# MishaLaskin/vqvae

Hardware: AMD Instinct MI355X
Metric: images/sec VQ-VAE forward (32x32x3, K=512, D=64) (higher is better)
Workload: dtype f32 (fp32 in/out/accumulate; conv products from two fp16 terms per operand, <= 2^-21 rel per product); 1 GPU; BASELINE config 3: full HIP path (Encoder+VQ+Decoder), 32x32x3, K=512, D=64; per_gpu_batch=4096, global_batch=4096, K=512, D=64, parallelism=batch-sharded replicas x1, no collective

## Files before the change

### vqvae_amd/csrc/conv_fused.hip

```cpp
#include "conv_host.h"

namespace vqvae {
#ifndef VQVAE_MID_SHFL_BPERMUTE
constexpr bool kSwz = true;
#else
constexpr bool kSwz = false;
#endif
#ifndef CRP_NW
#define CRP_NW 4
#endif
#ifndef CRP_MINW
#define CRP_MINW 2
#endif
struct DecHeadArgs {
    FrontConv fc;
    const u32x4 *w1img, *w2img;
    const int *hdr1, *hdr2;
    int flags;
    float *out;
    int *out_amax;
};
template <int NT3, bool VQ = false, bool GATHER = false, bool ZEOUT = false, bool DECHEAD = false>
__global__ __launch_bounds__(CRP_NW * 64, CRP_MINW) void conv_res_pair8_h2_kernel(const float *__restrict__ in, FrontConv fc,
                                                                   const u32x4 *__restrict__ w1img, const u32x4 *__restrict__ w2img,
                                                                   float *__restrict__ out, int B, int flags,
                                                                   const int *__restrict__ hdr1, const int *__restrict__ hdr2,
                                                                   const int *__restrict__ in_amax, int *__restrict__ out_amax,
                                                                   const u32x4 *__restrict__ w3img, const int *__restrict__ hdr3,
                                                                   const float *__restrict__ bias3, float *__restrict__ out3,
                                                                   int *__restrict__ zero_buf, int zero_n, VqFuse vq, DecHeadArgs dh) {
    static_assert(!DECHEAD || (VQ && !GATHER && !ZEOUT), "the decoder's head continues the quantizing instance");
    static_assert(NT3 == 0 || NT3 == 1 || NT3 == 2 || NT3 == 4, "the 1x1 post conv streams through NT3 weight stages of 16 KiB");
    static_assert(!VQ || (NT3 == 2 && CRP_NW == 4), "the fused quantizer takes the 64-channel z_e of four images per workgroup");
    constexpr int NT2 = 4, C = 128, MT = 2, PX = 64, HP = PX + 1, PLANE = HP * 2;
    constexpr int TILE4 = 2 * 2 * PLANE;
    constexpr int RBUF = 4 * HP;
    __shared__ u32x4 As_all[CRP_NW * TILE4];
    constexpr int WBUF = 18 * 64;
    const int nvq = VQ ? (vq.K32 >> 7) : 0;
    int NSTAGE = 18 + NT3 + nvq;
    FrontConv fcc = fc;
    const u32x4 *w1c = w1img, *w2c = w2img;
    __shared__ u32x4 Wb_all[2 * WBUF];
    __shared__ __attribute__((aligned(16))) unsigned char vq_tab_all[VQ ? CRP_NW * 1040 : 16];
    __shared__ int vq_hist_s[VQ ? 1024 : 1];
    __shared__ __attribute__((aligned(16))) float dw_s[288 + 32 * (NT3 > 0 ? NT3 : 1)];
    for (int i = threadIdx.x; i < 288 + 32 * NT3; i += CRP_NW * 64)
        dw_s[i] = i < 128 ? h2_dw(fc.hdr)[i] : (i < 160 ? h2_dw(hdr1)[i - 128] : (i < 288 ? h2_dw(hdr2)[i - 160] : h2_dw(hdr3)[i - 288]));
    __shared__ double vq_red_s[VQ ? CRP_NW : 1];
    if constexpr (VQ) {
        for (int i = threadIdx.x; i < vq.K; i += CRP_NW * 64) vq_hist_s[i] = 0;
    }
    const int tid = threadIdx.x, wave = tid >> 6;
    int lane, l31, h;
    u32x4 *As;
    float *Hs;
    unsigned dma_lane;
    int spx[MT];
    unsigned tapok[MT], tapok0[MT];
    const bool relu_out = flags & kFlagReluOut;
    constexpr int cpt = C >> 5;

    const long long img = (long long)blockIdx.x * CRP_NW + wave;
    const bool img_ok = img < B;
    if (zero_buf && blockIdx.x == 0)
        for (int i = tid; i < zero_n; i += CRP_NW * 64) zero_buf[i] = 0;

    auto lane_setup = [&](int t_id) {
        lane = t_id & 63;
        l31 = lane & 31;
        h = lane >> 5;
        As = As_all + (t_id >> 6) * TILE4;
        Hs = reinterpret_cast<float *>(As);
        dma_lane = (unsigned)lane * 16u;
#pragma unroll
        for (int mt = 0; mt < MT; ++mt) {
            spx[mt] = 32 * mt + l31;
            const int y = spx[mt] >> 3, x = spx[mt] & 7;
            unsigned m = 0;
#pragma unroll
            for (int t = 0; t < 9; ++t) {
                const int yy = y + t / 3 - 1, xx = x + t % 3 - 1;
                if (yy >= 0 && yy < 8 && xx >= 0 && xx < 8) m |= 1u << t;
            }
            tapok[mt] = m;
        }
    };
    lane_setup(tid);
    auto front_masks = [&]() {
#pragma unroll
        for (int mt = 0; mt < MT; ++mt) {
            const int y = spx[mt] >> 3, x = spx[mt] & 7;
            unsigned m0 = 0;
#pragma unroll
            for (int t = 0; t < 9; ++t) {
                const int y0 = y + (int)((fcc.dym >> (4 * t)) & 15) - 8, x0 = x + (int)((fcc.dxm >> (4 * t)) & 15) - 8;
                if (y0 >= 0 && y0 < 8 && x0 >= 0 && x0 < 8) m0 |= 1u << t;
            }
            tapok0[mt] = m0;
        }
    };
    front_masks();

    f32x16 Y[MT][NT2];
    const int wave_u = __builtin_amdgcn_readfirstlane(wave);
    auto dma = [&](const u32x4 *src_uniform, u32x4 *dst_piece) {
        const unsigned lds = __builtin_amdgcn_readfirstlane((unsigned)(unsigned long long)(__attribute__((address_space(3))) char *)(char *)dst_piece);
        asm volatile("s_mov_b32 m0, %2\n\ts_nop 0\n\tglobal_load_lds_dwordx4 %0, %1" ::"v"(dma_lane), "s"(src_uniform), "s"(lds) : "memory");
    };
    auto dma_slice = [&](int sl, int buf) {
        const u32x4 *base = w1c + (size_t)(sl >> 1) * 256 + (sl & 1) * 64;
        for (int p = wave_u; p < 18; p += CRP_NW)
            dma(base + (size_t)(p >> 1) * cpt * 256 + (p & 1) * 128, Wb_all + buf * WBUF + p * 64);
    };
    auto dma_linear = [&](const u32x4 *src, int buf) {
#pragma unroll
        for (int j = 0; j < 16 / CRP_NW; ++j) dma(src + (wave_u * (16 / CRP_NW) + j) * 64, Wb_all + buf * WBUF + (wave_u * (16 / CRP_NW) + j) * 64);
    };
    auto dma_stage = [&](int k, int buf) {
        if (VQ && k >= 18 + NT3) {
            const int j = k - (18 + NT3);
            dma_linear(reinterpret_cast<const u32x4 *>(vq.imgf) + (size_t)j * 1024, buf);
            if (wave_u == 0) dma(reinterpret_cast<const u32x4 *>(vq.seeds) + (size_t)j * 32, Wb_all + buf * WBUF + 16 * 64);
        }
        else if (k >= 18) dma_linear(w3img + (size_t)(k - 18) * 1024, buf);
        else if (k % 9 == 8) dma_linear(w2c, buf);
        else dma_slice(k % 9, buf);
    };
    auto dma_wait_sync = [&]() {
        asm volatile("s_waitcnt vmcnt(0)" ::: "memory");
        __syncthreads();
    };
    float ymax = 0.0f;
    int wstage = 0;
    f32x4 zr[2][8];
    f32x16(&Yo)[MT][NT2] = Y;
    float &ymax_o = ymax;
    int &wstage_o = wstage;
    auto front = [&](auto FZ) __attribute__((always_inline)) {
        constexpr bool FROMZ = decltype(FZ)::value;
        const FrontConv &fc = fcc;
        f32x16 Y[MT][NT2];
        float ymax = 0.0f;
        int wstage = 0;
        const int cpt0 = FROMZ ? 2 : fc.Cin >> 5;
        const float *src = in + ((size_t)(img_ok ? img : 0) * PX + lane) * fc.Cin;
        bool gbad = false;
        if constexpr (GATHER) {
            const long long k = vq.idx[(size_t)(img_ok ? img : 0) * PX + lane];
            gbad = k < 0 || k >= vq.K;
            src = in + (size_t)(gbad ? 0 : k) * fc.Cin;
        }
        const bool gany = GATHER && __builtin_amdgcn_ballot_w64(gbad) != 0;
        f32x4 raw[8];
        auto load_raw0 = [&](int cc) {
            if constexpr (FROMZ) {
#pragma unroll
                for (int j = 0; j < 8; ++j) raw[j] = cc == 0 ? zr[0][j] : zr[1][j];
                return;
            }
#pragma unroll
            for (int j = 0; j < 8; ++j) raw[j] = *reinterpret_cast<const f32x4 *>(src + 32 * cc + 4 * j);
            if (gany) {
                const float qn = __builtin_nanf("");
#pragma unroll
                for (int j = 0; j < 8; ++j) if (gbad) raw[j] = f32x4{qn, qn, qn, qn};
            }
        };
        float m = 0.0f;
        const int given = (!FROMZ && in_amax && img_ok) ? in_amax[img] : -1;
        auto fold_raw = [&]() {
#pragma unroll
            for (int j = 0; j < 8; ++j)
                m = fmaxf(m, fmaxf(fmaxf(__builtin_fabsf(raw[j].x), __builtin_fabsf(raw[j].y)), fmaxf(__builtin_fabsf(raw[j].z), __builtin_fabsf(raw[j].w))));
        };
        if constexpr (FROMZ) {
            load_raw0(0); fold_raw();
            load_raw0(1); fold_raw();
        } else if (given >= 0) m = __int_as_float(given);
        else for (int cc = 0; cc < cpt0; ++cc) {
            load_raw0(cc);
            fold_raw();
        }
        const int kx = wave_scale_exp<kSwz>(img_ok ? m : 0.0f);
        const float xs = __builtin_ldexpf(1.0f, kx), d0 = __builtin_ldexpf(1.0f, -kx);
#pragma unroll
        for (int mt = 0; mt < MT; ++mt)
#pragma unroll
            for (int nt = 0; nt < NT2; ++nt)
#pragma unroll
                for (int r = 0; r < 16; ++r) Y[mt][nt][r] = 0.0f;
        if (lane < 8) As[(lane >> 1) * PLANE + (lane & 1) * HP + PX] = u32x4{0, 0, 0, 0};
        auto dma_front = [&](int cc, int tap, int buf) {
            const u32x4 *base = fc.wimg + (size_t)(tap * cpt0 + cc) * (NT2 * 256);
#pragma unroll
            for (int j = 0; j < 16 / CRP_NW; ++j) {
                const int p = wave_u * (16 / CRP_NW) + j;
                dma(base + (p >> 2) * 256 + ((p >> 1) & 1) * 64 + (p & 1) * 128, Wb_all + buf * WBUF + p * 64);
            }
        };
        load_raw0(0);
        dma_front(0, 0, 0);
        for (int cc = 0; cc < cpt0; ++cc) {
            __builtin_amdgcn_wave_barrier();
            u32x4 *dst = As + lane;
#pragma unroll
            for (int t = 0; t < 2; ++t)
#pragma unroll
                for (int hh = 0; hh < 2; ++hh) {
                    u32x4 t1, t2;
                    split8_h(raw[4 * hh + 2 * t], raw[4 * hh + 2 * t + 1], xs, t1, t2);
                    dst[(t * 2 + 0) * PLANE + hh * HP] = t1;
                    dst[(t * 2 + 1) * PLANE + hh * HP] = t2;
                }
            lds_order_wave();
#pragma unroll 1
            for (int tap = 0; tap < 9; ++tap, ++wstage) {
                const int shift = ((int)((fc.dym >> (4 * tap)) & 15) - 8) * 8 + ((int)((fc.dxm >> (4 * tap)) & 15) - 8);
                u32x4 X[2][MT][2];
#pragma unroll
                for (int t = 0; t < 2; ++t)
#pragma unroll
                    for (int mt = 0; mt < MT; ++mt) {
                        const int p = ((tapok0[mt] >> tap) & 1u) ? spx[mt] + shift : PX;
                        const u32x4 *ap = As + (t * 2) * PLANE + h * HP + p;
                        X[t][mt][0] = ap[0];
                        X[t][mt][1] = ap[PLANE];
                    }
                if (!FROMZ && tap == 1 && cc + 1 < cpt0) {
                    asm volatile("s_waitcnt vmcnt(8)" ::: "memory");
                    __syncthreads();
                } else dma_wait_sync();
                if (tap + 1 < 9) dma_front(cc, tap + 1, (wstage + 1) & 1);
                else if (cc + 1 < cpt0) dma_front(cc + 1, 0, (wstage + 1) & 1);
                else dma_stage(0, (wstage + 1) & 1);
                if (tap == 0 && cc + 1 < cpt0) load_raw0(FROMZ ? 1 : cc + 1);
                const u32x4 *wt = Wb_all + (wstage & 1) * WBUF + lane;
                u32x4 Wc0 = wt[0], Wc1 = wt[64];
#pragma unroll
                for (int g = 0; g < 8; ++g) {
                    const int t = g >> 2, nt = g & 3;
                    u32x4 Wn0 = Wc0, Wn1 = Wc1;
                    if (g + 1 < 8) {
                        const u32x4 *bp = wt + (((g + 1) & 3) * 4 + ((g + 1) >> 2) * 2) * 64;
                        Wn0 = bp[0];
                        Wn1 = bp[64];
                    }
                    __builtin_amdgcn_sched_barrier(0);
                    prod3x2t(X[t][0][0], X[t][0][1], X[t][1][0], X[t][1][1], Wc0, Wc1, Y[0][nt], Y[1][nt]);
                    __builtin_amdgcn_sched_barrier(0);
                    Wc0 = Wn0;
                    Wc1 = Wn1;
                }
            }
        }
#pragma unroll
        for (int nt = 0; nt < NT2; ++nt)
#pragma unroll
            for (int g = 0; g < 4; ++g) {
                f32x4 bv = {0.0f, 0.0f, 0.0f, 0.0f};
                if (fc.bias) bv = *reinterpret_cast<const f32x4 *>(fc.bias + nt * 32 + 8 * g + 4 * h);
                const f32x4 dv = h2_dw4(dw_s, nt * 32, g, h, d0);
#pragma unroll
                for (int mt = 0; mt < MT; ++mt)
#pragma unroll
                    for (int q = 0; q < 4; q += 2)
                        SCALE2_BIAS_RELU2(Y[mt][nt][4 * g + q], Y[mt][nt][4 * g + q + 1], dv[q], dv[q + 1], bv[q], bv[q + 1], ymax);
            }
        lds_order_wave();
#pragma unroll
        for (int mt = 0; mt < MT; ++mt)
#pragma unroll
            for (int nt = 0; nt < NT2; ++nt) Yo[mt][nt] = Y[mt][nt];
        ymax_o = ymax;
        wstage_o = wstage;
    };
    front(std::false_type{});

    auto stage_sync = [&](int k) -> const u32x4 * {
        dma_wait_sync();
        if (k + 1 < NSTAGE) dma_stage(k + 1, (wstage + k + 1) & 1);
        return Wb_all + ((wstage + k) & 1) * WBUF + lane;
    };
    f32x16 acc1[MT];
    auto taps = [&](const u32x4 *wb, const u32x4 *pl) {
        u32x4 Xc[MT][2], Wc[2];
        auto ld = [&](int tap, u32x4(&X)[MT][2], u32x4(&W)[2]) {
            const int shift = (tap / 3 - 1) * 8 + (tap % 3 - 1);
#pragma unroll
            for (int mt = 0; mt < MT; ++mt) {
                const int p = ((tapok[mt] >> tap) & 1u) ? spx[mt] + shift : PX;
                X[mt][0] = pl[p];
                X[mt][1] = pl[p + HP * 2];
            }
            W[0] = wb[tap * 128];
            W[1] = wb[tap * 128 + 64];
        };
        ld(0, Xc, Wc);
#pragma unroll
        for (int tap = 0; tap < 9; ++tap) {
            u32x4 Xn[MT][2], Wn[2];
            if (tap + 1 < 9) ld(tap + 1, Xn, Wn);
            __builtin_amdgcn_sched_barrier(0);
            prod3x2t(Xc[0][0], Xc[0][1], Xc[1][0], Xc[1][1], Wc[0], Wc[1], acc1[0], acc1[1]);
            __builtin_amdgcn_sched_barrier(0);
            if (tap + 1 < 9) {
#pragma unroll
                for (int mt = 0; mt < MT; ++mt) { Xc[mt][0] = Xn[mt][0]; Xc[mt][1] = Xn[mt][1]; }
                Wc[0] = Wn[0]; Wc[1] = Wn[1];
            }
        }
    };
    auto put_planes = [&](int buf, const u32x4(&T1)[MT][2], const u32x4(&T2)[MT][2], int t) {
        u32x4 *pb = As + buf * RBUF + h * HP + l31;
#pragma unroll
        for (int mt = 0; mt < MT; ++mt) {
            pb[32 * mt] = T1[mt][t];
            pb[32 * mt + 2 * HP] = T2[mt][t];
        }
    };
    auto layer = [&](auto LT, bool relu_after) __attribute__((always_inline)) {
        constexpr int LI = decltype(LT)::value;
        const int kx = wave_scale_exp<kSwz>(img_ok ? ymax : 0.0f);
        const float xscale = __builtin_ldexpf(1.0f, kx), d1 = __builtin_ldexpf(1.0f, -kx);
#pragma unroll
        for (int mt = 0; mt < MT; ++mt)
#pragma unroll
            for (int r = 0; r < 16; ++r) acc1[mt][r] = 0.0f;
        u32x4 T1[MT][2], T2[MT][2];
#pragma unroll
        for (int mt = 0; mt < MT; ++mt) acc_to_ksteps(Y[mt][0], xscale, T1[mt], T2[mt]);
        __builtin_amdgcn_wave_barrier();
        put_planes(0, T1, T2, 0);
#pragma unroll
        for (int c = 0; c < NT2; ++c) {
            __builtin_amdgcn_wave_barrier();
            put_planes(1, T1, T2, 1);
            lds_order_wave();
            taps(stage_sync(9 * LI + 2 * c), As + h * HP);
            if (c + 1 < NT2) {
#pragma unroll
                for (int mt = 0; mt < MT; ++mt) acc_to_ksteps(Y[mt][c + 1], xscale, T1[mt], T2[mt]);
                __builtin_amdgcn_wave_barrier();
                put_planes(0, T1, T2, 0);
            }
            lds_order_wave();
            taps(stage_sync(9 * LI + 2 * c + 1), As + RBUF + h * HP);
        }
        float m = 0.0f;
#pragma unroll
        for (int g = 0; g < 4; ++g) {
            const f32x4 dv = h2_dw4(dw_s + 128, 0, g, h, d1);
#pragma unroll
            for (int mt = 0; mt < MT; ++mt)
#pragma unroll
                for (int q = 0; q < 4; q += 2)
                    SCALE2_BIAS_RELU2(acc1[mt][4 * g + q], acc1[mt][4 * g + q + 1], dv[q], dv[q + 1], 0.0f, 0.0f, m);
        }
        const int kh = wave_scale_exp<kSwz>(m);
        const float hscale = __builtin_ldexpf(1.0f, kh), d2 = __builtin_ldexpf(1.0f, -kh);
        u32x4 H1[MT][2], Hb[MT][2];
#pragma unroll
        for (int mt = 0; mt < MT; ++mt) acc_to_ksteps(acc1[mt], hscale, H1[mt], Hb[mt]);
        const u32x4 *wb = stage_sync(9 * LI + 8);
        float nmax = 0.0f;
#pragma unroll
        for (int nt = 0; nt < NT2; ++nt) {
            u32x4 Wc[2][2];
#pragma unroll
            for (int t = 0; t < 2; ++t) { Wc[t][0] = wb[nt * 256 + t * 64]; Wc[t][1] = wb[nt * 256 + t * 64 + 128]; }
            f32x16 acc2[MT];
#pragma unroll
            for (int mt = 0; mt < MT; ++mt)
#pragma unroll
                for (int r = 0; r < 16; ++r) acc2[mt][r] = 0.0f;
#pragma unroll
            for (int t = 0; t < 2; ++t)
                prod3x2t(H1[0][t], Hb[0][t], H1[1][t], Hb[1][t], Wc[t][0], Wc[t][1], acc2[0], acc2[1]);
            if (relu_after) {
#pragma unroll
                for (int g = 0; g < 4; ++g) {
                    const f32x4 dv = h2_dw4(dw_s + 160, nt * 32, g, h, d2);
#pragma unroll
                    for (int mt = 0; mt < MT; ++mt)
#pragma unroll
                        for (int q = 0; q < 4; q += 2) {
                            const int r = 4 * g + q;
                            const float y0 = relu1(__builtin_fmaf(acc2[mt][r], dv[q], Y[mt][nt][r]));
                            const float y1 = relu1(__builtin_fmaf(acc2[mt][r + 1], dv[q + 1], Y[mt][nt][r + 1]));
                            Y[mt][nt][r] = y0;
                            Y[mt][nt][r + 1] = y1;
                            vmax3(nmax, y0, y1);
                        }
                }
            } else {
#pragma unroll
                for (int g = 0; g < 4; ++g) {
                    const f32x4 dv = h2_dw4(dw_s + 160, nt * 32, g, h, d2);
#pragma unroll
                    for (int mt = 0; mt < MT; ++mt)
#pragma unroll
                        for (int q = 0; q < 4; q += 2) {
                            const int r = 4 * g + q;
                            const float y0 = __builtin_fmaf(acc2[mt][r], dv[q], Y[mt][nt][r]), y1 = __builtin_fmaf(acc2[mt][r + 1], dv[q + 1], Y[mt][nt][r + 1]);
                            Y[mt][nt][r] = y0;
                            Y[mt][nt][r + 1] = y1;
                            vmax3_abs(nmax, y0, y1);
                        }
                }
            }
        }
        ymax = nmax;
    };
    layer(std::integral_constant<int, 0>{}, true);
    layer(std::integral_constant<int, 1>{}, relu_out);
    if (out_amax && img_ok) publish_amax_exclusive<kSwz>(out_amax, img, ymax, lane);

    auto store_tile = [&](const float(&v)[16], float *dst, int ld) {
        __builtin_amdgcn_wave_barrier();
#pragma unroll
        for (int g = 0; g < 4; ++g)
            *reinterpret_cast<f32x4 *>(Hs + l31 * 36 + 8 * g + 4 * h) = f32x4{v[4 * g], v[4 * g + 1], v[4 * g + 2], v[4 * g + 3]};
        lds_order_wave();
#pragma unroll
        for (int k = 0; k < 4; ++k) {
            const int p = (lane >> 3) + 8 * k;
            *reinterpret_cast<f32x4 *>(dst + (size_t)p * ld + 4 * (lane & 7)) = *reinterpret_cast<const f32x4 *>(Hs + p * 36 + 4 * (lane & 7));
        }
    };
    const long long wbase = img * PX;
    if constexpr (NT3 > 0) {
        const int kx3 = wave_scale_exp<kSwz>(img_ok ? ymax : 0.0f);
        const float xs3 = __builtin_ldexpf(1.0f, kx3), d3 = __builtin_ldexpf(1.0f, -kx3);
        f32x16 acc3[MT][NT3];
#pragma unroll
        for (int mt = 0; mt < MT; ++mt)
#pragma unroll
            for (int n3 = 0; n3 < NT3; ++n3)
#pragma unroll
                for (int r = 0; r < 16; ++r) acc3[mt][n3][r] = 0.0f;
        const u32x4 *wb = nullptr;
#pragma unroll
        for (int c = 0; c < NT2; ++c) {
            u32x4 T1[MT][2], T2[MT][2];
#pragma unroll
            for (int mt = 0; mt < MT; ++mt) acc_to_ksteps(Y[mt][c], xs3, T1[mt], T2[mt]);
            constexpr int CPS = 4 / NT3;
            if (c % CPS == 0) wb = stage_sync(18 + c / CPS);
#pragma unroll
            for (int t = 0; t < 2; ++t)
#pragma unroll
                for (int n3 = 0; n3 < NT3; ++n3) {
                    const u32x4 *bp = wb + ((c % CPS) * NT3 + n3) * 256 + t * 64;
                    prod3x2t(T1[0][t], T2[0][t], T1[1][t], T2[1][t], bp[0], bp[128], acc3[0][n3], acc3[1][n3]);
                }
        }
        if constexpr (VQ) {
#pragma unroll
            for (int mt = 0; mt < MT; ++mt)
#pragma unroll
                for (int n3 = 0; n3 < NT3; ++n3)
#pragma unroll
                    for (int g = 0; g < 4; ++g) {
                        f32x4 bv = {0.0f, 0.0f, 0.0f, 0.0f};
                        if (bias3) bv = *reinterpret_cast<const f32x4 *>(bias3 + n3 * 32 + 8 * g + 4 * h);
                        const f32x4 dv = h2_dw4(dw_s + 288, n3 * 32, g, h, d3);
#pragma unroll
                        for (int q = 0; q < 4; ++q) acc3[mt][n3][4 * g + q] = acc3[mt][n3][4 * g + q] * dv[q] + bv[q];
                    }
            u32x4 zb[MT][4];
            float zn2[MT];
#pragma unroll
            for (int mt = 0; mt < MT; ++mt) {
                float sq = 0.0f;
#pragma unroll
                for (int n3 = 0; n3 < NT3; ++n3)
#pragma unroll
                    for (int t = 0; t < 2; ++t) {
                        float P[4], Q[4];
#pragma unroll
                        for (int q = 0; q < 4; ++q) {
                            P[q] = acc3[mt][n3][4 * t + q];
                            Q[q] = acc3[mt][n3][8 + 4 * t + q];
                            swap_halves(P[q], Q[q]);
                        }
                        u32x4 v;
                        v.x = __builtin_bit_cast(unsigned, __builtin_convertvector((f32x2v{P[0], P[1]}), f16x2));
                        v.y = __builtin_bit_cast(unsigned, __builtin_convertvector((f32x2v{P[2], P[3]}), f16x2));
                        v.z = __builtin_bit_cast(unsigned, __builtin_convertvector((f32x2v{Q[0], Q[1]}), f16x2));
                        v.w = __builtin_bit_cast(unsigned, __builtin_convertvector((f32x2v{Q[2], Q[3]}), f16x2));
                        zb[mt][2 * n3 + t] = v;
                        sq = sqsum8_f16(v.x, v.y, v.z, v.w, sq);
                    }
                const auto sw = __builtin_amdgcn_permlane32_swap(__float_as_uint(sq), __float_as_uint(sq), false, false);
                zn2[mt] = sq + __uint_as_float(h ? sw[0] : sw[1]);
            }
            const float inf = __builtin_inff();
            const float pinf = inf, ninf = -inf;
            unsigned keymask = trk::kKeyMask;
            asm volatile("" : "+v"(keymask));
            trk::Lane L[MT];
#pragma unroll
            for (int mt = 0; mt < MT; ++mt) trk::init(L[mt], ninf);
            auto sweep_stage = [&](const u32x4 *wb, const float *sd, int j, auto &&use) {
#pragma unroll
                for (int ctl = 0; ctl < 4; ++ctl) {
                    f32x16 seed;
#pragma unroll
                    for (int g = 0; g < 4; ++g) {
                        const f32x4 e4 = *reinterpret_cast<const f32x4 *>(sd + ctl * 32 + h * 16 + 4 * g);
                        seed[4 * g] = e4.x; seed[4 * g + 1] = e4.y; seed[4 * g + 2] = e4.z; seed[4 * g + 3] = e4.w;
                    }
                    u32x4 a[4];
#pragma unroll
                    for (int ks = 0; ks < 4; ++ks) a[ks] = wb[ctl * 256 + ks * 64];
                    use(4 * j + ctl, a, seed);
                }
            };
            for (int j = 0; j < nvq; ++j) {
                const u32x4 *wb = stage_sync(18 + NT3 + j);
                const float *sd = reinterpret_cast<const float *>(wb - lane + 16 * 64);
                sweep_stage(wb, sd, j, [&](int ct, const u32x4(&a)[4], const f32x16 &seed) {
                    f32x16 acc[MT];
#pragma unroll
                    for (int mt = 0; mt < MT; ++mt) {
                        acc[mt] = __builtin_amdgcn_mfma_f32_32x32x16_f16(__builtin_bit_cast(f16x8, a[0]), __builtin_bit_cast(f16x8, zb[mt][0]), seed, 0, 0, 0);
#pragma unroll
                        for (int ks = 1; ks < 4; ++ks)
                            acc[mt] = __builtin_amdgcn_mfma_f32_32x32x16_f16(__builtin_bit_cast(f16x8, a[ks]), __builtin_bit_cast(f16x8, zb[mt][ks]), acc[mt], 0, 0, 0);
                    }
                    unsigned cell0 = (unsigned)(2 * ct), cell1 = cell0 + 1u;
                    asm volatile("" : "+s"(cell0), "+s"(cell1));
#pragma unroll
                    for (int mt = 0; mt < MT; ++mt) trk::tile(L[mt], acc[mt], cell0, cell1, keymask, ninf, pinf);
                });
            }
            vqu::Tables tb = vqu::tables(vq_tab_all + wave_u * 1040);
            const vqu::BoundP bound = vqu::load_boundp(vq.flags);
            vqu::RowsSp<MT> R;
            vqu::classify_sp<MT>(L, zn2, bound, vq.K, lane, img_ok ? PX : 0, ninf, tb.task_s, R);
            vqu::Flagged FL = vqu::exact_begin_sp<MT>(R, lane, tb);
            int ntasks = FL.ndirect;
            const bool rescan_me = FL.hmask && FL.ndirect <= 64;
            int nres = 0;
            if (__syncthreads_or(rescan_me ? 1 : 0)) {
                dma_stage(18 + NT3, 0);
                for (int j = 0; j < nvq; ++j) {
                    dma_wait_sync();
                    if (j + 1 < nvq) dma_stage(18 + NT3 + j + 1, (j + 1) & 1);
                    if (rescan_me && FL.ndirect + nres <= 64) {
                        const u32x4 *wb = Wb_all + (j & 1) * WBUF + lane;
                        const float *sd = reinterpret_cast<const float *>(Wb_all + (j & 1) * WBUF + 16 * 64);
#pragma unroll
                        for (int mt = 0; mt < MT; ++mt)
                            if ((unsigned)(FL.hmask >> (32 * mt))) {
                                const float thr_t = (((unsigned)(FL.hmask >> (32 * mt)) >> l31) & 1u) ? R.thr[mt] : inf;
                                sweep_stage(wb, sd, j, [&](int ct, const u32x4(&a)[4], const f32x16 &seed) {
                                    f32x16 acc = __builtin_amdgcn_mfma_f32_32x32x16_f16(__builtin_bit_cast(f16x8, a[0]), __builtin_bit_cast(f16x8, zb[mt][0]), seed, 0, 0, 0);
#pragma unroll
                                    for (int ks = 1; ks < 4; ++ks)
                                        acc = __builtin_amdgcn_mfma_f32_32x32x16_f16(__builtin_bit_cast(f16x8, a[ks]), __builtin_bit_cast(f16x8, zb[mt][ks]), acc, 0, 0, 0);
                                    vqu::rescan_tile(acc, thr_t, ct, mt, lane, vq.K, FL.ndirect, ninf, tb, nres);
                                });
                            }
                    }
                }
                if (rescan_me) {
                    lds_order_wave();
                    ntasks = FL.ndirect + nres;
                }
            }
            __syncthreads();
            unsigned char *zlo = reinterpret_cast<unsigned char *>(As);
            unsigned char *zhi = reinterpret_cast<unsigned char *>(Wb_all) + (size_t)wave_u * 9216;
            auto zchunk = [&](int row, int c16) -> f32x4 * {
                unsigned char *b = row < 32 ? zlo + row * 256 : zhi + (row - 32) * 256;
                return reinterpret_cast<f32x4 *>(b + (((unsigned)c16 ^ ((unsigned)row & 15u)) << 4));
            };
            __builtin_amdgcn_wave_barrier();
#pragma unroll
            for (int mt = 0; mt < MT; ++mt)
#pragma unroll
                for (int n3 = 0; n3 < NT3; ++n3)
#pragma unroll
                    for (int g = 0; g < 4; ++g)
                        *zchunk(32 * mt + l31, 8 * n3 + 2 * g + h) = f32x4{acc3[mt][n3][4 * g], acc3[mt][n3][4 * g + 1], acc3[mt][n3][4 * g + 2], acc3[mt][n3][4 * g + 3]};
            lds_order_wave();
            if constexpr (ZEOUT) {
                if (img_ok)
#pragma unroll
                    for (int c16 = 0; c16 < 16; ++c16)
                        *reinterpret_cast<f32x4 *>(out3 + ((size_t)img * PX + lane) * 64 + 4 * c16) = *zchunk(lane, c16);
            }
            vqu::exact_end_sp<MT>(R, FL, ntasks, lane, tb, vq.cb, vq.ee, vq.K,
                           [&](int rr, int jc) { return *zchunk(rr, jc); },
                           [&](int rr, int c) { return reinterpret_cast<const float *>(zchunk(rr, c >> 2))[c & 3]; });
            const int j16 = lane & 15, g4 = lane >> 4;
            float sacc;
            if constexpr (DECHEAD) {
                sacc = vqu::epilogue_sp<false, MT>(R, lane, vq.cb, vq.K, [&](int t, int i) { return *zchunk(32 * t + 4 * i + g4, j16); },
                                                   nullptr, img_ok ? PX : 0, vq.idx + (size_t)(img_ok ? img : 0) * PX, vq_hist_s, nullptr, 0, 0u,
                                                   [&](int t, int i, const f32x4 &o) { *zchunk(32 * t + 4 * i + g4, j16) = o; });
                lds_order_wave();
#pragma unroll
                for (int c16 = 0; c16 < 16; ++c16) zr[c16 >> 3][c16 & 7] = *zchunk(lane, c16);
            } else
            sacc = vqu::epilogue_sp<false, MT>(R, lane, vq.cb, vq.K, [&](int t, int i) { return *zchunk(32 * t + 4 * i + g4, j16); },
                                             (img_ok && vq.zq) ? vq.zq + (size_t)img * PX * 64 : nullptr, img_ok ? PX : 0,
                                             vq.idx + (size_t)(img_ok ? img : 0) * PX, vq_hist_s);
            double dacc = img_ok ? (double)sacc : 0.0;
            dacc = wave_sum_all<kSwz>(dacc);
            if (lane == 0) vq_red_s[wave_u] = dacc;
            __syncthreads();
            if (tid == 0) {
                double sum = 0.0;
                for (int w = 0; w < CRP_NW; ++w) sum += vq_red_s[w];
                vq.partials[blockIdx.x] = sum;
            }
            for (int k = tid; k < vq.K; k += CRP_NW * 64) {
                const int c = vq_hist_s[k];
                if (c) atomicAdd(&vq.hist[k], c);
            }
            if constexpr (DECHEAD) {
                int tid2 = tid;
                asm volatile("" : "+v"(tid2));
                lane_setup(tid2);
                fcc = dh.fc;
                w1c = dh.w1img;
                w2c = dh.w2img;
                NSTAGE = 18;
                for (int i = tid; i < 288; i += CRP_NW * 64)
                    dw_s[i] = i < 128 ? h2_dw(dh.fc.hdr)[i] : (i < 160 ? h2_dw(dh.hdr1)[i - 128] : h2_dw(dh.hdr2)[i - 160]);
                front_masks();
                front(std::true_type{});
                layer(std::integral_constant<int, 0>{}, true);
                layer(std::integral_constant<int, 1>{}, (dh.flags & kFlagReluOut) != 0);
                if (dh.out_amax && img_ok) publish_amax_exclusive<kSwz>(dh.out_amax, img, ymax, lane);
                if (img_ok) {
#pragma unroll
                    for (int mt = 0; mt < MT; ++mt)
#pragma unroll
                        for (int nt = 0; nt < NT2; ++nt) {
                            float v[16];
#pragma unroll
                            for (int r = 0; r < 16; ++r) v[r] = Y[mt][nt][r];
                            store_tile(v, dh.out + (wbase + mt * 32) * C + nt * 32, C);
                        }
                }
            }
        } else
// ... 739 lines not shown
```

Measured before the change: 4.530 million images/s.

## Carry last tap's MFMA product across stage barriers to overlap with weight DMA

In the fused residual-pair conv kernel, the final matrix product of each weight stage is deferred past the next stage's wait/barrier and DMA issue. It then runs while the next stage's weights are loaded. Operand loads for the next stage are issued before the barrier, and the stage wait now also drains LDS counters (lgkmcnt(0)). The aim is to hide barrier and DMA-issue latency behind MFMA work. This is enabled only for the VQ and NT3==0 instances, and it adds register pressure and more complex control flow.

```diff
diff --git a/vqvae_amd/csrc/conv_fused.hip b/vqvae_amd/csrc/conv_fused.hip
--- a/vqvae_amd/csrc/conv_fused.hip
+++ b/vqvae_amd/csrc/conv_fused.hip
@@ -5,6 +5,13 @@
 constexpr bool kSwz = true;
 #else
 constexpr bool kSwz = false;
+#endif
+#ifndef VQVAE_NO_STAGE_CARRY
+constexpr bool kCarry = true;
+#define STAGE_WAIT(vm) asm volatile("s_waitcnt vmcnt(" #vm ") lgkmcnt(0)" ::: "memory")
+#else
+constexpr bool kCarry = false;
+#define STAGE_WAIT(vm) asm volatile("s_waitcnt vmcnt(" #vm ")" ::: "memory")
 #endif
 #ifndef CRP_NW
 #define CRP_NW 4
@@ -33,6 +40,7 @@
     static_assert(NT3 == 0 || NT3 == 1 || NT3 == 2 || NT3 == 4, "the 1x1 post conv streams through NT3 weight stages of 16 KiB");
     static_assert(!VQ || (NT3 == 2 && CRP_NW == 4), "the fused quantizer takes the 64-channel z_e of four images per workgroup");
     constexpr int NT2 = 4, C = 128, MT = 2, PX = 64, HP = PX + 1, PLANE = HP * 2;
+    constexpr bool kC = kCarry && (VQ || NT3 == 0);
     constexpr int TILE4 = 2 * 2 * PLANE;
     constexpr int RBUF = 4 * HP;
     __shared__ u32x4 As_all[CRP_NW * TILE4];
@@ -128,7 +136,7 @@
         else dma_slice(k % 9, buf);
     };
     auto dma_wait_sync = [&]() {
-        asm volatile("s_waitcnt vmcnt(0)" ::: "memory");
+        STAGE_WAIT(0);
         __syncthreads();
     };
     float ymax = 0.0f;
@@ -201,6 +209,7 @@
         };
         load_raw0(0);
         dma_front(0, 0, 0);
+        u32x4 X[2][MT][2], Wc0, Wc1;
         for (int cc = 0; cc < cpt0; ++cc) {
             __builtin_amdgcn_wave_barrier();
             u32x4 *dst = As + lane;
@@ -217,9 +226,7 @@
 #pragma unroll 1
             for (int tap = 0; tap < 9; ++tap, ++wstage) {
                 const int shift = ((int)((fc.dym >> (4 * tap)) & 15) - 8) * 8 + ((int)((fc.dxm >> (4 * tap)) & 15) - 8);
-                u32x4 X[2][MT][2];
-#pragma unroll
-                for (int t = 0; t < 2; ++t)
+                auto ldX = [&](int t) {
 #pragma unroll
                     for (int mt = 0; mt < MT; ++mt) {
                         const int p = ((tapok0[mt] >> tap) & 1u) ? spx[mt] + shift : PX;
@@ -227,16 +234,33 @@
                         X[t][mt][0] = ap[0];
                         X[t][mt][1] = ap[PLANE];
                     }
+                };
+                ldX(0);
+                if constexpr (!kC) ldX(1);
                 if (!FROMZ && tap == 1 && cc + 1 < cpt0) {
-                    asm volatile("s_waitcnt vmcnt(8)" ::: "memory");
+                    STAGE_WAIT(8);
                     __syncthreads();
                 } else dma_wait_sync();
+                const u32x4 *wt = Wb_all + (wstage & 1) * WBUF + lane;
+                u32x4 Wf0, Wf1;
+                if constexpr (kC) { Wf0 = wt[0]; Wf1 = wt[64]; }
                 if (tap + 1 < 9) dma_front(cc, tap + 1, (wstage + 1) & 1);
                 else if (cc + 1 < cpt0) dma_front(cc + 1, 0, (wstage + 1) & 1);
                 else dma_stage(0, (wstage + 1) & 1);
                 if (tap == 0 && cc + 1 < cpt0) load_raw0(FROMZ ? 1 : cc + 1);
-                const u32x4 *wt = Wb_all + (wstage & 1) * WBUF + lane;
-                u32x4 Wc0 = wt[0], Wc1 = wt[64];
+                if constexpr (kC) {
+                    if (wstage > 0) {
+                        __builtin_amdgcn_sched_barrier(0);
+                        prod3x2t(X[1][0][0], X[1][0][1], X[1][1][0], X[1][1][1], Wc0, Wc1, Y[0][NT2 - 1], Y[1][NT2 - 1]);
+                        __builtin_amdgcn_sched_barrier(0);
+                    }
+                    ldX(1);
+                    Wc0 = Wf0;
+                    Wc1 = Wf1;
+                } else {
+                    Wc0 = wt[0];
+                    Wc1 = wt[64];
+                }
 #pragma unroll
                 for (int g = 0; g < 8; ++g) {
                     const int t = g >> 2, nt = g & 3;
@@ -247,13 +271,14 @@
                         Wn1 = bp[64];
                     }
                     __builtin_amdgcn_sched_barrier(0);
-                    prod3x2t(X[t][0][0], X[t][0][1], X[t][1][0], X[t][1][1], Wc0, Wc1, Y[0][nt], Y[1][nt]);
+                    if (!kC || g + 1 < 8) prod3x2t(X[t][0][0], X[t][0][1], X[t][1][0], X[t][1][1], Wc0, Wc1, Y[0][nt], Y[1][nt]);
                     __builtin_amdgcn_sched_barrier(0);
                     Wc0 = Wn0;
                     Wc1 = Wn1;
                 }
             }
         }
+        if constexpr (kC) prod3x2t(X[1][0][0], X[1][0][1], X[1][1][0], X[1][1][1], Wc0, Wc1, Y[0][NT2 - 1], Y[1][NT2 - 1]);
 #pragma unroll
         for (int nt = 0; nt < NT2; ++nt)
 #pragma unroll
@@ -283,9 +308,9 @@
         return Wb_all + ((wstage + k) & 1) * WBUF + lane;
     };
     f32x16 acc1[MT];
-    auto taps = [&](const u32x4 *wb, const u32x4 *pl) {
-        u32x4 Xc[MT][2], Wc[2];
-        auto ld = [&](int tap, u32x4(&X)[MT][2], u32x4(&W)[2]) {
+    auto taps = [&](int k, const u32x4 *pl, u32x4(&Xc)[MT][2], u32x4(&Wc)[2], bool carry_in, bool carry_out) {
+        const u32x4 *wb = nullptr;
+        auto ldx = [&](int tap, u32x4(&X)[MT][2]) {
             const int shift = (tap / 3 - 1) * 8 + (tap % 3 - 1);
 #pragma unroll
             for (int mt = 0; mt < MT; ++mt) {
@@ -293,22 +318,41 @@
                 X[mt][0] = pl[p];
                 X[mt][1] = pl[p + HP * 2];
             }
+        };
+        auto ldw = [&](int tap, u32x4(&W)[2]) {
             W[0] = wb[tap * 128];
             W[1] = wb[tap * 128 + 64];
         };
-        ld(0, Xc, Wc);
-#pragma unroll
-        for (int tap = 0; tap < 9; ++tap) {
-            u32x4 Xn[MT][2], Wn[2];
-            if (tap + 1 < 9) ld(tap + 1, Xn, Wn);
+        auto prod = [&]() {
             __builtin_amdgcn_sched_barrier(0);
             prod3x2t(Xc[0][0], Xc[0][1], Xc[1][0], Xc[1][1], Wc[0], Wc[1], acc1[0], acc1[1]);
             __builtin_amdgcn_sched_barrier(0);
-            if (tap + 1 < 9) {
-#pragma unroll
-                for (int mt = 0; mt < MT; ++mt) { Xc[mt][0] = Xn[mt][0]; Xc[mt][1] = Xn[mt][1]; }
-                Wc[0] = Wn[0]; Wc[1] = Wn[1];
-            }
+        };
+        auto rotate = [&](const u32x4(&Xn)[MT][2], const u32x4(&Wn)[2]) {
+#pragma unroll
+            for (int mt = 0; mt < MT; ++mt) { Xc[mt][0] = Xn[mt][0]; Xc[mt][1] = Xn[mt][1]; }
+            Wc[0] = Wn[0]; Wc[1] = Wn[1];
+        };
+        if constexpr (kC) {
+            u32x4 Xn[MT][2], Wn[2];
+            ldx(0, Xn);
+            dma_wait_sync();
+            wb = Wb_all + ((wstage + k) & 1) * WBUF + lane;
+            ldw(0, Wn);
+            if (k + 1 < NSTAGE) dma_stage(k + 1, (wstage + k + 1) & 1);
+            if (carry_in) prod();
+            rotate(Xn, Wn);
+        } else {
+            wb = stage_sync(k);
+            ldx(0, Xc);
+            ldw(0, Wc);
+        }
+#pragma unroll
+        for (int tap = 0; tap < 9; ++tap) {
+            u32x4 Xn[MT][2], Wn[2];
+            if (tap + 1 < 9) { ldx(tap + 1, Xn); ldw(tap + 1, Wn); }
+            if (tap + 1 < 9 || !carry_out) prod();
+            if (tap + 1 < 9) rotate(Xn, Wn);
         }
     };
     auto put_planes = [&](int buf, const u32x4(&T1)[MT][2], const u32x4(&T2)[MT][2], int t) {
@@ -332,12 +376,14 @@
         for (int mt = 0; mt < MT; ++mt) acc_to_ksteps(Y[mt][0], xscale, T1[mt], T2[mt]);
         __builtin_amdgcn_wave_barrier();
         put_planes(0, T1, T2, 0);
+        constexpr bool carry = kC;
+        u32x4 Xc[MT][2], Wc[2];
 #pragma unroll
         for (int c = 0; c < NT2; ++c) {
             __builtin_amdgcn_wave_barrier();
             put_planes(1, T1, T2, 1);
             lds_order_wave();
-            taps(stage_sync(9 * LI + 2 * c), As + h * HP);
+            taps(9 * LI + 2 * c, As + h * HP, Xc, Wc, carry && c > 0, false);
             if (c + 1 < NT2) {
 #pragma unroll
                 for (int mt = 0; mt < MT; ++mt) acc_to_ksteps(Y[mt][c + 1], xscale, T1[mt], T2[mt]);
@@ -345,7 +391,7 @@
                 put_planes(0, T1, T2, 0);
             }
             lds_order_wave();
-            taps(stage_sync(9 * LI + 2 * c + 1), As + RBUF + h * HP);
+            taps(9 * LI + 2 * c + 1, As + RBUF + h * HP, Xc, Wc, false, carry && c + 1 < NT2);
         }
         float m = 0.0f;
 #pragma unroll
```

Result: no change. 4.561 million images/s, median of 6 (+0.7%).
